# zhengyk19/vit-rpe-rope

Measured on AMD Instinct MI355X. Metric: train images/sec, CIFAR-10 ViT d=192 L=6 H=6, higher is better.
Workload: dtype bf16; 1 GPU; CIFAR-10-shaped 32x32 patch4 ViT d=192 L=6 H=6, --pos_encoding rope-axial theta=100, bf16, full train step (fwd+CE+bwd+AdamW), random-init weights; per_gpu_batch=512, global_batch=512, parallelism=dp1, hip_graph=True

## Files before the change

include/vitpe_debug.h:

```cpp
#ifndef VITPE_DEBUG_H
#define VITPE_DEBUG_H
#include "vitpe.h"
#ifdef __cplusplus
extern "C" {
#endif

int vitpe_selftest_mma(int dtype, const void* A, const void* Bt, const void* Brow, float* C_row,
                       float* C_tr, vitpe_stream_t stream);

int vitpe_debug_wgrad_census(int dtype, const vitpe_wgrad_problem* problems, int nprob, unsigned long long* census,
                             vitpe_stream_t stream);
int vitpe_debug_attn_census(const void* xn, const void* wqkv, void* out, const float* cos, const float* sin,
                            int B, unsigned long long* census, vitpe_stream_t stream);
int vitpe_debug_attn32_census(const void* xn, const void* wqkv_wide, void* out, const float* cos, const float* sin,
                              int B, unsigned long long* census, vitpe_stream_t stream);
int vitpe_debug_tail2_census(const void* attn_out, const void* x_in, const void* Wp_packed, const float* bp,
                             const float* gamma, const float* beta, void* x_mid, float* mean2, float* rstd2,
                             void* xn_out, const void* W1_packed, const float* b1, const void* W2_packed,
                             const float* b2, void* gp_out, void* h_out, void* out, float* mean_out, float* rstd_out,
                             int M, int HID, unsigned long long* census, vitpe_stream_t stream);
int vitpe_debug_set_gemm2d_mt(int mt);
int vitpe_debug_set_wgrad_wide(int on);
int vitpe_debug_read_bw(const void* src, long long bytes, int depth, int workgroups, unsigned* sink, vitpe_stream_t stream);
#ifdef __cplusplus
}
#endif
#endif
```

vit-rpe-rope_amd/csrc/wgrad.hip:

```cpp
#include "common.h"
#include <stdlib.h>

namespace vitpe {

constexpr int WG_MAXPROB = 28;
constexpr int WG_BLK = 192;

struct WgProb {
  const void* dY;
  const void* X;
  float* dW;
  float* dbias;
  const float* xmean;
  const float* xrstd;
  const float* xgamma;
  const float* xbeta;
  int M, N, K;
  int xop;
  int rs;
  int unit0;
  int nbn;
  int stages;
};
constexpr int WG_TABLE = 512;
struct WgArgs {
  int nprob, total_units, units_per_wg;
  int use_table;
  int nranges;
  int full_rounds, total_blocks;
  int tail_rounds;
  int bk;
  int nbig;
  int short_slots;
  int range_major;
  unsigned long long* census;
  WgProb p[WG_MAXPROB];
  unsigned short table[WG_TABLE];
};
static_assert(sizeof(WgArgs) <= 4096, "kernel argument block");
constexpr int WG_CENSUS_STAGES = 24, WG_CENSUS_SLOTS = 4;
constexpr int WG_SHORT_SPR = 2;

template <typename T> struct WgLayout;
template <> struct WgLayout<bf16> {
  static constexpr int LD = WG_BLK;
  static __device__ __forceinline__ int chunk(int r, int cc) {
    const int s = ((r >> 1) & 1) | (((r >> 3) & 1) << 1);
    return r * LD + ((((cc >> 1) ^ s)) << 4) + ((cc & 1) << 3);
  }
  static __device__ __forceinline__ Frag<bf16> tr(const bf16* tile, int rb0, int rb1, int c0) { return tr_ld<LD>(tile, rb0, rb1, c0); }
  template <int LD>
  static __device__ __forceinline__ Frag<bf16> tr_ld(const bf16* tile, int rb0, int rb1, int c0) {
    const int i = threadIdx.x & 15, q = i >> 2, p = i & 3;
    typedef __attribute__((address_space(3))) s16x4 lds_s16x4;
    const int r0 = rb0 + q, r1 = rb1 + q;
    constexpr int PAR = (LD % 128 == 0) ? 4 : 0;
    const int s0 = (((r0 >> 1) & 1) | (((r0 >> 3) & 1) << 1)) ^ ((r0 & 1) * PAR), s1 = (((r1 >> 1) & 1) | (((r1 >> 3) & 1) << 1)) ^ ((r1 & 1) * PAR);
    const bf16* a0 = tile + r0 * LD + (((c0 >> 4) ^ s0) << 4) + 4 * p;
    const bf16* a1 = tile + r1 * LD + (((c0 >> 4) ^ s1) << 4) + 4 * p;
    s16x4 lo = __builtin_amdgcn_ds_read_tr16_b64_v4i16((lds_s16x4*)a0);
    s16x4 hi = __builtin_amdgcn_ds_read_tr16_b64_v4i16((lds_s16x4*)a1);
    const s16x8 both = __builtin_shufflevector(lo, hi, 0, 1, 2, 3, 4, 5, 6, 7);
    Frag<bf16> f;
    f.v = __builtin_bit_cast(bf16x8, both);
    return f;
  }
};
template <> struct WgLayout<float> {
  static constexpr int LD = WG_BLK + 4;
  static __device__ __forceinline__ int chunk(int r, int cc) { return r * LD + cc * 4; }
  static __device__ __forceinline__ Frag<float> tr(const float* tile, int rb0, int rb1, int c0) {
    return ld_frag_tr(tile, LD, rb0, rb1, c0);
  }
};

template <class RunFn>
VITPE_DEV void wg_dispatch_placed(const WgArgs& a, RunFn run);

template <class RunFn>
VITPE_DEV void wg_dispatch(const WgArgs& a, RunFn run) {
  wg_dispatch_placed(a, run);
  for (int s = blockIdx.x; s < a.short_slots; s += gridDim.x) {
    int q = s, pi = a.nbig;
    for (int i = a.nbig; i < a.nprob - 1; ++i) {
      const int nsl = a.p[i].nbn * ((a.p[i].K + a.bk - 1) / a.bk) * ((a.p[i].stages + WG_SHORT_SPR - 1) / WG_SHORT_SPR);
      if (pi == i && q >= nsl) { q -= nsl; pi = i + 1; }
    }
    const WgProb& P = a.p[pi];
    const int nr = (P.stages + WG_SHORT_SPR - 1) / WG_SHORT_SPR;
    const int ub = P.unit0 + (q / nr) * P.stages, u0 = ub + (q % nr) * WG_SHORT_SPR;
    run(u0, min(ub + P.stages, u0 + WG_SHORT_SPR));
  }
}

template <class RunFn>
VITPE_DEV void wg_dispatch_placed(const WgArgs& a, RunFn run) {
  if (a.use_table == 2) {
    const int G = gridDim.x, idx = (blockIdx.x & 7) * (G >> 3) + (blockIdx.x >> 3);
    const int nrounds = a.range_major ? a.full_rounds : a.full_rounds + a.tail_rounds;
    for (int r = 0; r < nrounds; ++r) {
      int gb, rng = 0, R = 1;
      if (a.range_major) {
        const int vb = r * G + idx;
        R = a.nranges;
        rng = vb / a.total_blocks;
        gb = rng < R ? vb - rng * a.total_blocks : a.total_blocks;
      } else if (r < a.full_rounds) {
        gb = r * G + idx;
      } else {
        R = a.nranges;
        const int rem = a.total_blocks - a.full_rounds * G, q = (r - a.full_rounds) * G + idx;
        if (q >= rem * R) continue;
        rng = q / rem;
        gb = a.full_rounds * G + q % rem;
      }
      if (gb >= a.total_blocks) continue;
      int pi = 0, b0 = 0;
      for (int i = 0; i < a.nbig; ++i) {
        const int nb = a.p[i].nbn * ((a.p[i].K + a.bk - 1) / a.bk);
        if (gb >= b0 + nb) { b0 += nb; pi = i + 1; } else break;
      }
      const WgProb& P = a.p[pi];
      const int spr = (P.stages + R - 1) / R;
      const int ub = P.unit0 + (gb - b0) * P.stages;
      const int u0 = ub + min(P.stages, rng * spr), uend = ub + min(P.stages, (rng + 1) * spr);
      if (u0 < uend) run(u0, uend);
    }
    return;
  }
  int u0, uend;
  if (a.use_table == 1) {
    const unsigned ent = a.table[blockIdx.x];
    if (ent == 0xFFFFu) return;
    const WgProb& P = a.p[ent >> 11];
    const int blk = (int)((ent >> 5) & 0x3Fu), rng = (int)(ent & 0x1Fu);
    const int spr = (P.stages + a.nranges - 1) / a.nranges;
    u0 = P.unit0 + blk * P.stages + min(P.stages, rng * spr);
    uend = P.unit0 + blk * P.stages + min(P.stages, (rng + 1) * spr);
  } else {
    u0 = blockIdx.x * a.units_per_wg;
    uend = min(a.total_units, u0 + a.units_per_wg);
  }
  if (u0 >= uend) return;
  run(u0, uend);
}

template <typename T, bool CENSUS, bool LNX>
__global__ __launch_bounds__(768) void wgrad_group_kernel(WgArgs a) {
  using LY = WgLayout<T>;
  constexpr int RPS = 128 / (int)sizeof(T);
  constexpr int CPS = RPS / 32;
  constexpr int CHN = CH<T>::n;
  constexpr int CPR = WG_BLK / CHN;
  static_assert(RPS * CPR == 2 * 768, "a slab is two chunks per thread");
  constexpr int SLAB = RPS * LY::LD;
  __shared__ __attribute__((aligned(16))) T sm[2 * 2 * SLAB];

  const int tid = threadIdx.x, lane = tid & 63, c = lane & 15, g = lane >> 4;
  const int wave = __builtin_amdgcn_readfirstlane(tid >> 6);
  const int wn = wave / 3, wk = wave % 3;

  struct Cur {
    const T* dY; const T* X; float* dW; float* dbias;
    const float* xmean; const float* xrstd; const float* xgamma; const float* xbeta;
    int M, N, K, n0, k0, stage, stages, xop, rs;
  };
  auto decode = [&](int u, Cur& s) {
    int pi = 0;
    for (int i = 1; i < a.nprob; ++i) pi = (u >= a.p[i].unit0) ? i : pi;
    const WgProb& P = a.p[pi];
    const int ub = u - P.unit0, blk = ub / P.stages;
    s.dY = reinterpret_cast<const T*>(P.dY); s.X = reinterpret_cast<const T*>(P.X); s.dW = P.dW; s.dbias = P.dbias;
    s.M = P.M; s.N = P.N; s.K = P.K; s.stages = P.stages;
    s.xmean = P.xop ? P.xmean : reinterpret_cast<const float*>(P.dY);
    s.xrstd = P.xop ? P.xrstd : reinterpret_cast<const float*>(P.dY);
    s.xgamma = P.xgamma; s.xbeta = P.xbeta; s.xop = P.xop; s.rs = P.rs;
    s.stage = ub - blk * P.stages;
    s.n0 = (blk % P.nbn) * WG_BLK;
    s.k0 = (blk / P.nbn) * a.bk;
  };

  const Chunk16 zero = {0u, 0u, 0u, 0u};
  Chunk16 rg[4];
  float lnA[2], lnB[2];
  bool ln_staged = false;
  auto gload = [&](const Cur& s) {
    const int mb = s.stage * RPS;
    ln_staged = LNX && s.xop == 1;
#pragma unroll
    for (int i = 0; i < 4; ++i) {
      const int q = tid + 768 * (i & 1), row = q / CPR, cc = q % CPR;
      const int gm = mb + row;
      if (i < 2) {
        const int gn = s.n0 + cc * CHN;
        rg[i] = (gm < s.M && gn < s.N) ? *reinterpret_cast<const Chunk16*>(s.dY + (size_t)gm * s.rs * s.N + gn) : zero;
      } else {
        const int gk = s.k0 + cc * CHN;
        const bool ok = gm < s.M && gk < s.K;
        rg[i] = ok ? *reinterpret_cast<const Chunk16*>(s.X + (size_t)gm * s.rs * s.K + gk) : zero;
        if (LNX) {
          const size_t gs = (s.xop == 1) ? (size_t)min(gm, s.M - 1) * s.rs : 0;
          lnA[i - 2] = s.xrstd[gs];
          lnB[i - 2] = s.xmean[gs];
        }
      }
    }
  };
  auto sstore = [&](int buf) {
#pragma unroll
    for (int i = 0; i < 4; ++i) {
      const int q = tid + 768 * (i & 1), row = q / CPR, cc = q % CPR;
      Chunk16 v = rg[i];
      if (LNX && i >= 2 && ln_staged) {
        float f[CHN];
        chunk_to_f32<T>(v, f);
        const float rs = lnA[i - 2], nb = -lnB[i - 2] * rs;
#pragma unroll
        for (int t = 0; t < CHN; ++t) f[t] = fmaf(f[t], rs, nb);
        v = f32_to_chunk<T>(f);
      }
      *reinterpret_cast<Chunk16*>(sm + (buf * 2 + (i >> 1)) * SLAB + LY::chunk(row, cc)) = v;
    }
  };

  f32x4 acc[3][4], accb[3];
  auto clear = [&]() {
#pragma unroll
    for (int nt = 0; nt < 3; ++nt) {
      accb[nt] = (f32x4){0.f, 0.f, 0.f, 0.f};
#pragma unroll
      for (int kt = 0; kt < 4; ++kt) acc[nt][kt] = (f32x4){0.f, 0.f, 0.f, 0.f};
    }
  };
  Frag<T> ones;
#pragma unroll
  for (int t = 0; t < 8; ++t) ones.v[t] = from_f32<T>(1.0f);

  auto compute = [&](int buf, bool bias) {
    const T* sY = sm + (buf * 2 + 0) * SLAB;
    const T* sX = sm + (buf * 2 + 1) * SLAB;
#pragma unroll
    for (int cs = 0; cs < CPS; ++cs) {
      const int rb0 = cs * 32 + 8 * g, rb1 = rb0 + 4;
      Frag<T> fy[3], fx[4];
#pragma unroll
      for (int nt = 0; nt < 3; ++nt) fy[nt] = LY::tr(sY, rb0, rb1, wn * 48 + 16 * nt);
#pragma unroll
      for (int kt = 0; kt < 4; ++kt) fx[kt] = LY::tr(sX, rb0, rb1, wk * 64 + 16 * kt);
#pragma unroll
      for (int nt = 0; nt < 3; ++nt)
#pragma unroll
        for (int kt = 0; kt < 4; ++kt) mma(fy[nt], fx[kt], acc[nt][kt]);
      if (bias) {
#pragma unroll
        for (int nt = 0; nt < 3; ++nt) mma(fy[nt], ones, accb[nt]);
      }
    }
  };
  auto flush = [&](const Cur& s, bool bias) {
    float gam[4], bet[4];
#pragma unroll
    for (int kt = 0; kt < 4; ++kt) {
      const int gk = s.k0 + wk * 64 + 16 * kt + c;
      gam[kt] = (LNX && s.xop == 1 && gk < s.K) ? s.xgamma[gk] : 1.f;
      bet[kt] = (LNX && s.xop == 1 && gk < s.K) ? s.xbeta[gk] : 0.f;
    }
#pragma unroll
    for (int nt = 0; nt < 3; ++nt)
#pragma unroll
      for (int r = 0; r < 4; ++r) {
        const int gn = s.n0 + wn * 48 + 16 * nt + 4 * g + r;
#pragma unroll
        for (int kt = 0; kt < 4; ++kt) {
          const int gk = s.k0 + wk * 64 + 16 * kt + c;
          float v = acc[nt][kt][r];
          if (LNX && s.xop == 1) v = fmaf(v, gam[kt], bet[kt] * accb[nt][r]);
          if (gn < s.N && gk < s.K) atomicAdd(s.dW + (size_t)gn * s.K + gk, v);
        }
        if (bias && c == 0 && gn < s.N) atomicAdd(s.dbias + gn, accb[nt][r]);
      }
    clear();
  };

  bool first_run = true;
  auto run = [&](int u0, int uend) {
    if (!first_run) __syncthreads();
    first_run = false;
  Cur cur, nxt;
    decode(u0, cur);
    gload(cur);
    clear();
    auto stamp = [&](int u, int slot) {
      if (CENSUS && lane == 0 && u - u0 < WG_CENSUS_STAGES)
        a.census[(((size_t)blockIdx.x * 12 + wave) * WG_CENSUS_STAGES + (u - u0)) * WG_CENSUS_SLOTS + slot] = __builtin_amdgcn_s_memtime();
    };
    for (int u = u0; u < uend; ++u) {
      const int buf = (u - u0) & 1;
      sstore(buf);
      stamp(u, 0);
      nxt = cur;
      bool flush_now = (u + 1 == uend);
      if (u + 1 < uend) {
        if (cur.stage + 1 < cur.stages) nxt.stage = cur.stage + 1;
        else { decode(u + 1, nxt); flush_now = true; }
        gload(nxt);
      }
      stamp(u, 2);
      __syncthreads();
      stamp(u, 1);
      const bool bias = (cur.dbias != nullptr) && cur.k0 == 0 && wk == 0;
      compute(buf, bias || (LNX && cur.xop == 1));
      stamp(u, 3);
      if (flush_now) flush(cur, bias);
      cur = nxt;
    }
  };

  wg_dispatch(a, run);
}

constexpr int WW_BK = 384, WW_TH = 512;

__global__ __launch_bounds__(WW_TH) void wgrad_wide_kernel(WgArgs a) {
  using T = bf16;
  using LY = WgLayout<bf16>;
  constexpr int RPS = 64, YLD = WG_BLK, XLD = WW_BK;
  constexpr int YSLAB = RPS * YLD, XSLAB = RPS * XLD, STG = YSLAB + XSLAB;
  constexpr int YI = YSLAB / 512, XI = XSLAB / 512, NI = (YI + XI) / 8;
  static_assert((YI + XI) % 8 == 0, "instructions per wave");
  __shared__ __attribute__((aligned(1024))) T sm[2 * STG];

  const int tid = threadIdx.x, lane = tid & 63, c = lane & 15, g = lane >> 4;
  const int wave = __builtin_amdgcn_readfirstlane(tid >> 6);
  const int wn = wave >> 2, wk = wave & 3;

  struct Cur { const T* dY; const T* X; float* dW; float* dbias; int M, N, K, n0, k0, stage, stages; };
  auto decode = [&](int u, Cur& s) {
    int pi = 0;
    for (int i = 1; i < a.nprob; ++i) pi = (u >= a.p[i].unit0) ? i : pi;
    const WgProb& P = a.p[pi];
    const int ub = u - P.unit0, blk = ub / P.stages;
    s.dY = reinterpret_cast<const T*>(P.dY); s.X = reinterpret_cast<const T*>(P.X); s.dW = P.dW; s.dbias = P.dbias;
    s.M = P.M; s.N = P.N; s.K = P.K; s.stages = P.stages;
    s.stage = ub - blk * P.stages;
    s.n0 = (blk % P.nbn) * WG_BLK;
    s.k0 = (blk / P.nbn) * WW_BK;
  };
  auto swz = [](int r, int cl) { return ((((cl >> 1) ^ (((r >> 1) & 1) | (((r >> 3) & 1) << 1))) << 1) | (cl & 1)); };
  auto swzx = [](int r, int cl) {
    return ((((cl >> 1) ^ ((((r >> 1) & 1) | (((r >> 3) & 1) << 1)) ^ ((r & 1) << 2))) << 1) | (cl & 1));
  };
  static_assert(YI == 24 && XI == 48, "instruction j of a wave: j < 3 -> dY slab, else X slab");
  const unsigned sm_lds = (unsigned)(uintptr_t)(__attribute__((address_space(3))) void*)sm;
  auto dma = [&](const Cur& s, int buf) {
    const int mb = s.stage * RPS;
    int ln = lane;
    asm volatile("" : "+v"(ln));
#pragma unroll
    for (int j = 0; j < NI; ++j) {
      const int q = wave + 8 * j;
      const T* src;
      if (j < 3) {
        const int p = q * 64 + ln, r = p / (YLD / 8), cl = p % (YLD / 8);
        src = s.dY + (size_t)min(mb + r, s.M - 1) * s.N + s.n0 + swz(r, cl) * 8;
      } else {
        const int p = (q - YI) * 64 + ln, r = p / (XLD / 8), cl = p % (XLD / 8);
        src = s.X + (size_t)min(mb + r, s.M - 1) * s.K + s.k0 + swzx(r, cl) * 8;
      }
      const unsigned dst = sm_lds + (unsigned)(buf * STG + q * 512) * 2;
      unsigned keep;
      asm volatile("s_mov_b32 %0, m0\n\ts_mov_b32 m0, %2\n\ts_nop 0\n\tglobal_load_lds_dwordx4 %1, off\n\ts_mov_b32 m0, %0"
                   : "=&s"(keep) : "v"(src), "s"(dst) : "memory");
    }
  };

  f32x4 acc[6][6], accb[2];
  auto clear = [&]() {
    accb[0] = accb[1] = (f32x4){0.f, 0.f, 0.f, 0.f};
#pragma unroll
    for (int nt = 0; nt < 6; ++nt)
#pragma unroll
      for (int kt = 0; kt < 6; ++kt) acc[nt][kt] = (f32x4){0.f, 0.f, 0.f, 0.f};
  };
  Frag<T> ones;
#pragma unroll
  for (int t = 0; t < 8; ++t) ones.v[t] = from_f32<T>(1.0f);

  auto compute = [&](int buf, bool bias) {
    const T* sY = sm + buf * STG;
    const T* sX = sY + YSLAB;
#pragma unroll
    for (int cs = 0; cs < 2; ++cs) {
      const int rb0 = cs * 32 + 8 * g, rb1 = rb0 + 4;
      __builtin_amdgcn_sched_barrier(0);
      Frag<T> fy[6];
#pragma unroll
      for (int nt = 0; nt < 6; ++nt) fy[nt] = LY::tr_ld<YLD>(sY, rb0, rb1, wn * 96 + 16 * nt);
#pragma unroll
      for (int h = 0; h < 2; ++h) {
        Frag<T> fx[3];
#pragma unroll
        for (int t = 0; t < 3; ++t) fx[t] = LY::tr_ld<XLD>(sX, rb0, rb1, wk * 96 + 16 * (3 * h + t));
#pragma unroll
        for (int nt = 0; nt < 6; ++nt)
#pragma unroll
          for (int t = 0; t < 3; ++t) mma(fy[nt], fx[t], acc[nt][3 * h + t]);
        __builtin_amdgcn_sched_barrier(0);
      }
      if (bias) {
        if (wk == 0) { mma(fy[0], ones, accb[0]); mma(fy[1], ones, accb[1]); }
        else if (wk == 1) { mma(fy[2], ones, accb[0]); mma(fy[3], ones, accb[1]); }
        else { mma(fy[4], ones, accb[0]); mma(fy[5], ones, accb[1]); }
      }
    }
  };
  auto flush = [&](const Cur& s, bool bias) {
#pragma unroll
    for (int nt = 0; nt < 6; ++nt)
#pragma unroll
      for (int r = 0; r < 4; ++r) {
        const int gn = s.n0 + wn * 96 + 16 * nt + 4 * g + r;
        float* row = s.dW + (size_t)gn * s.K + s.k0 + wk * 96 + c;
#pragma unroll
        for (int kt = 0; kt < 6; ++kt) atomicAdd(row + 16 * kt, acc[nt][kt][r]);
      }
    if (bias && c == 0) {
#pragma unroll
      for (int t = 0; t < 2; ++t)
#pragma unroll
        for (int r = 0; r < 4; ++r) atomicAdd(s.dbias + s.n0 + wn * 96 + 16 * (2 * wk + t) + 4 * g + r, accb[t][r]);
    }
    clear();
  };

  bool first_run = true;
  auto run = [&](int u0, int uend) {
    if (!first_run) __syncthreads();
    first_run = false;
    Cur cur, nxt;
    decode(u0, cur);
    dma(cur, 0);
    clear();
    for (int u = u0; u < uend; ++u) {
      const int buf = (u - u0) & 1;
      __builtin_amdgcn_s_waitcnt(0x0F70);
      __syncthreads();
      if (cur.stage * RPS + RPS > cur.M) {
        const int first = cur.M - cur.stage * RPS;
        T* sY = sm + buf * STG;
        for (int q = tid; q < (RPS - first) * (YLD / 8); q += WW_TH)
          *reinterpret_cast<Chunk16*>(sY + first * YLD + q * 8) = (Chunk16){0u, 0u, 0u, 0u};
        __syncthreads();
      }
      nxt = cur;
      bool flush_now = (u + 1 == uend);
      if (u + 1 < uend) {
        if (cur.stage + 1 < cur.stages) nxt.stage = cur.stage + 1;
        else { decode(u + 1, nxt); flush_now = true; }
        dma(nxt, buf ^ 1);
      }
      const bool bias = (cur.dbias != nullptr) && cur.k0 == 0 && wk < 3;
      compute(buf, bias);
      if (flush_now) flush(cur, bias);
      cur = nxt;
    }
  };
  wg_dispatch(a, run);
}

}

using namespace vitpe;

struct vitpe_wgrad_problem_abi {
  const void* dY;
  const void* X;
  float* dW;
  float* dbias;
  int M, N, K, x_op;
  const float* x_mean;
  const float* x_rstd;
  const float* x_gamma;
  const float* x_beta;
};

static int wgrad_cu_count() {
  static int n = 0;
  if (n == 0) {
    int dev = 0, v = 0;
    if (hipGetDevice(&dev) != hipSuccess || hipDeviceGetAttribute(&v, hipDeviceAttributeMultiprocessorCount, dev) != hipSuccess || v <= 0)
      v = 256;
    n = v;
  }
  return n;
}

static int wgrad_group_launch(int dtype, const void* problems, const int* row_step, int nprob, unsigned long long* census,
                              hipStream_t stream);
static bool g_wide_ok = true;
extern "C" int vitpe_debug_set_wgrad_wide(int on) { g_wide_ok = on != 0; return 0; }

extern "C" int vitpe_wgrad_group(int dtype, const void* problems, int nprob, hipStream_t stream) {
  return wgrad_group_launch(dtype, problems, nullptr, nprob, nullptr, stream);
}

extern "C" int vitpe_wgrad_group_rows(int dtype, const void* problems, const int* row_step, int nprob, hipStream_t stream) {
  return wgrad_group_launch(dtype, problems, row_step, nprob, nullptr, stream);
}

extern "C" int vitpe_debug_wgrad_census(int dtype, const void* problems, int nprob, unsigned long long* census,
                                        hipStream_t stream) {
  VITPE_REQUIRE(census != nullptr && dtype == 1);
  return wgrad_group_launch(dtype, problems, nullptr, nprob, census, stream);
}

static int wgrad_group_launch(int dtype, const void* problems, const int* row_step, int nprob, unsigned long long* census,
                              hipStream_t stream) {
  VITPE_REQUIRE(problems && nprob >= 0 && nprob <= WG_MAXPROB && (dtype == 0 || dtype == 1));
  const vitpe_wgrad_problem_abi* pr = reinterpret_cast<const vitpe_wgrad_problem_abi*>(problems);
  const int RPS = dtype == 1 ? 64 : 32, CHN = dtype == 1 ? 8 : 4;
  WgArgs a{};
  a.census = census;
  bool wide = g_wide_ok && dtype == 1 && census == nullptr && nprob > 0;
  for (int i = 0; i < nprob; ++i)
    wide = wide && (pr[i].M == 0 || (pr[i].x_op == 0 && pr[i].N % WG_BLK == 0 && pr[i].K % WW_BK == 0 &&
                                     (row_step == nullptr || row_step[i] <= 1)));
  a.bk = wide ? WW_BK : WG_BLK;
  int max_stages = 0;
  for (int i = 0; i < nprob; ++i) max_stages = (pr[i].M + RPS - 1) / RPS > max_stages ? (pr[i].M + RPS - 1) / RPS : max_stages;
  int units = 0, np = 0, nbig = 0;
  for (int pass = 0; pass < 2; ++pass) {
    for (int i = 0; i < nprob; ++i) {
      const vitpe_wgrad_problem_abi& p = pr[i];
      VITPE_REQUIRE(p.dY && p.X && p.dW && p.M >= 0 && p.N > 0 && p.K > 0 && p.N % CHN == 0 && p.K % CHN == 0);
      VITPE_REQUIRE(row_step == nullptr || row_step[i] >= 1);
      if (p.M == 0) continue;
      const int stages = (p.M + RPS - 1) / RPS;
      if ((stages * 8 <= max_stages) != (pass == 1)) continue;
      WgProb& q = a.p[np++];
      VITPE_REQUIRE(p.x_op == 0 || (p.x_op == 1 && p.x_mean && p.x_rstd && p.x_gamma && p.x_beta));
      q.dY = p.dY; q.X = p.X; q.dW = p.dW; q.dbias = p.dbias; q.M = p.M; q.N = p.N; q.K = p.K;
      q.xop = p.x_op; q.xmean = p.x_mean; q.xrstd = p.x_rstd; q.xgamma = p.x_gamma; q.xbeta = p.x_beta;
      q.rs = row_step != nullptr ? row_step[i] : 1;
      q.unit0 = units;
      q.nbn = (p.N + WG_BLK - 1) / WG_BLK;
      q.stages = stages;
      const long long nu = (long long)q.nbn * ((p.K + a.bk - 1) / a.bk) * q.stages;
      VITPE_REQUIRE(units + nu < (1LL << 30));
      units += (int)nu;
    }
    if (pass == 0) nbig = np;
  }
  if (units == 0) return 0;
  a.nprob = np;
  a.nbig = nbig;
  a.total_units = units;
  const int np_all = np;
  np = nbig;
  const int ncu = wgrad_cu_count();
  int grid = 0;
  int total_blocks = 0, max_blocks = 0, min_stages = 1 << 30;
  for (int i = 0; i < np; ++i) {
    const int nb = a.p[i].nbn * ((a.p[i].K + a.bk - 1) / a.bk);
    total_blocks += nb;
    max_blocks = nb > max_blocks ? nb : max_blocks;
    min_stages = a.p[i].stages < min_stages ? a.p[i].stages : min_stages;
  }
  int R = (2 * ncu) / (total_blocks > 0 ? total_blocks : 1);
  if (R > 255) R = 255;
  if (R >= 2 && R <= 8 && R <= min_stages / 4 && max_blocks <= 63 && np <= 31) {
    int len[8] = {0, 0, 0, 0, 0, 0, 0, 0};
    bool fits = true;
    for (int i = 0; i < WG_TABLE; ++i) a.table[i] = 0xFFFFu;
    for (int r = 0; r < R && fits; ++r)
      for (int i = 0; i < np && fits; ++i) {
        const int nb = a.p[i].nbn * ((a.p[i].K + a.bk - 1) / a.bk);
        int x = 0;
        for (int k = 1; k < 8; ++k) x = len[k] < len[x] ? k : x;
        for (int b = 0; b < nb; ++b) {
          const int id = (len[x] + b) * 8 + x;
          if (id >= WG_TABLE) { fits = false; break; }
          a.table[id] = (unsigned short)(((unsigned)i << 11) | ((unsigned)b << 5) | (unsigned)r);
        }
        len[x] += nb;
      }
    if (fits) {
      int mx = 0;
      for (int k = 0; k < 8; ++k) mx = len[k] > mx ? len[k] : mx;
      a.use_table = 1;
      a.nranges = R;
      grid = mx * 8;
    }
  }
  const int G = ncu & ~7;
  if (!a.use_table && G >= 8 && total_blocks >= G) {
    a.use_table = 2;
    a.total_blocks = total_blocks;
    a.full_rounds = total_blocks / G;
    const int rem = total_blocks - a.full_rounds * G;
    int bestR = 1, bestT = rem > 0 ? 1 : 0;
    int Rmax = min_stages / 4;
    if (Rmax > 8) Rmax = 8;
    for (int Rc = 2; rem > 0 && Rc <= Rmax; ++Rc) {
      const int Tc = (rem * Rc + G - 1) / G;
      if ((long long)Tc * bestR < (long long)bestT * Rc) { bestR = Rc; bestT = Tc; }
    }
    a.nranges = bestR;
    a.tail_rounds = bestT;
    grid = G;
  }
  if (!a.use_table && G >= 8 && total_blocks > 0 && total_blocks < G) {
    int bestR = 0, bestk = 0;
    double besteff = 0.0;
    for (int k = 1; k <= 3; ++k) {
      int Rk = (k * G) / total_blocks;
      if (Rk > min_stages / 4) Rk = min_stages / 4;
      if (Rk > 31) Rk = 31;
      if (Rk < 2) continue;
      const double eff = (double)total_blocks * Rk / (double)(((total_blocks * Rk + G - 1) / G) * G);
      if (eff > besteff + 1e-9) { besteff = eff; bestR = Rk; bestk = k; }
    }
    if (bestR >= 2 && besteff >= 0.97) {
      a.use_table = 2;
      a.range_major = 1;
      a.total_blocks = total_blocks;
      a.nranges = bestR;
      a.full_rounds = (total_blocks * bestR + G - 1) / G;
      grid = G;
      (void)bestk;
    }
  }
  if (a.use_table) {
    for (int i = nbig; i < np_all; ++i)
      a.short_slots += a.p[i].nbn * ((a.p[i].K + a.bk - 1) / a.bk) * ((a.p[i].stages + WG_SHORT_SPR - 1) / WG_SHORT_SPR);
  }
  np = np_all;
  if (!a.use_table) {
    const int wgs = units < ncu ? units : ncu;
    a.units_per_wg = (units + wgs - 1) / wgs;
    grid = (units + a.units_per_wg - 1) / a.units_per_wg;
  }
  bool lnx = false;
  for (int i = 0; i < np; ++i) lnx = lnx || a.p[i].xop != 0;
  if (census != nullptr) VITPE_REQUIRE(!lnx && dtype == 1);
  if (wide) hipLaunchKernelGGL(wgrad_wide_kernel, dim3(grid), dim3(WW_TH), 0, stream, a);
  else if (census != nullptr) hipLaunchKernelGGL((wgrad_group_kernel<bf16, true, false>), dim3(grid), dim3(768), 0, stream, a);
  else if (dtype == 1 && lnx) hipLaunchKernelGGL((wgrad_group_kernel<bf16, false, true>), dim3(grid), dim3(768), 0, stream, a);
  else if (dtype == 1) hipLaunchKernelGGL((wgrad_group_kernel<bf16, false, false>), dim3(grid), dim3(768), 0, stream, a);
  else if (lnx) hipLaunchKernelGGL((wgrad_group_kernel<float, false, true>), dim3(grid), dim3(768), 0, stream, a);
  else hipLaunchKernelGGL((wgrad_group_kernel<float, false, false>), dim3(grid), dim3(768), 0, stream, a);
  VITPE_CHECK_LAUNCH();
}
```

vit-rpe-rope_amd/vitpe/engine.py:

```python
from __future__ import annotations

import contextlib
import dataclasses
import math
import os
from typing import Dict, List, Optional

import numpy as np
import torch
import torch.distributed as dist
import torch.nn as nn

from . import _lib as L
from . import ddp
from . import kernels as K
from .positional_encoding import (AbsolutePositionalEncoding, PolynomialRPE, RelativePositionalEncoding, RoPEAxial,
                                  RoPEMixed)
from .head import StepHead
from .optim import StepOptimizer
from .route import (ALIGN, KIND_FRAG, KIND_FRAG_PHI, KIND_QKV, KIND_QKV_WIDE, KIND_T, Route, resolve_route,
                    shadow_plan)
from .vit import VisionTransformer

SITE_ATTN, SITE_PROJ, SITE_MLP1, SITE_MLP2, SITE_PATH_A, SITE_PATH_M = range(6)
SITES_PER_LAYER = 6


def site_row(layer: int, site: int) -> int:
    return SITES_PER_LAYER * layer + site


def shift_rng_offsets(table: torch.Tensor, rank: int) -> torch.Tensor:
    inc = (int(rank) << 48) & 0xFFFFFFFFFFFFFFFF
    out = table.clone()
    out[:, 1] += inc - (1 << 64) if inc >= (1 << 63) else inc
    return out


def new_augment_rng(device, rank: int = 0) -> torch.Tensor:
    return shift_rng_offsets(K.new_rng_pairs(1, device), rank)


def engine_unsupported(model):
    active = []
    for blk in model.blocks:
        if blk.attn.qkv.bias is not None:
            active.append("qkv_bias")
        if blk.attn.attn_drop_p > 0.:
            active.append("attn_drop")
        if blk.attn.proj_drop_p > 0. or blk.mlp.drop > 0.:
            active.append("drop")
        if blk.drop_path_p > 0.:
            active.append("drop_path")
    return sorted(set(active))


class TrainEngine:
    def __init__(self, model: VisionTransformer, batch_size: int, compute_dtype=torch.bfloat16, lr=1e-3,
                 weight_decay=0.01, betas=(0.9, 0.999), eps=1e-8, process_group=None, use_graph=True, fuse_ln=None,
                 extras=False):
        active = engine_unsupported(model)
        if active and not extras:
            raise NotImplementedError("TrainEngine does not support " + ", ".join(active) + " (the fused training path has "
                                      "no qkv bias and no dropout); train this model through the module path instead.  "
                                      "TrainEngine(..., extras=True) runs them on the per-Linear route")
        dev = next(model.parameters()).device
        if dev.type != "cuda":
            raise L.VitpeError("TrainEngine needs the model on the HIP device (no CPU path)")
        self.model, self.dev, self.T, self.B = model, dev, compute_dtype, batch_size
        self.pg = process_group
        self.world = dist.get_world_size(process_group) if (dist.is_available() and dist.is_initialized()) else 1
        self.use_graph = use_graph
        m = model
        self.D, self.H, self.Lyr, self.p = m.embed_dim, m.num_heads, len(m.blocks), m.patch_size
        self.C, self.P, self.Cn = m.patch_embed.weight.shape[1], m.num_patches, m.num_classes
        self.N, self.grid = self.P + 1, int(math.sqrt(self.P))
        self.S, self.M = self.grid * self.p, self.B * self.N
        self.hid = m.blocks[0].mlp.fc1.weight.shape[0]
        self.route: Route = resolve_route(compute_dtype, self.C, self.S, self.p, self.D, self.H, self.hid, self.Lyr, self.Cn,
                                          extras=extras, fuse_ln=fuse_ln)
        self.__dict__.update(dataclasses.asdict(self.route))
        self._save_hidden = True
        self._build_flat(lr, weight_decay, betas, eps)
        self._build_buffers()
        self._build_rng_table()
        self.aug_rng, self.aug_pad, self.aug_hflip = None, 0, False
        self.split_layer = max(1, self.Lyr // 2)
        self.bucket_off = self._off[id(next(self.model.blocks[self.split_layer].parameters()))] \
            if self.Lyr >= 2 else 0
        self.overlap_comm = self.world > 1 and self.Lyr >= 2
        self.allpairs = (ddp.AllPairsSum(self.pg) if self.world > 1 and os.environ.get("VITPE_DDP_ALLPAIRS", "0") == "1"
                         else None)
        self._comm_stream = torch.cuda.Stream(device=dev) if self.allpairs is not None else None
        self.ddp_graph = self.world > 1 and os.environ.get("VITPE_DDP_GRAPH", "0") == "1"
        self._drop_graphs()
        self.steps_done = 0

    def _drop_graphs(self):
        self.graph_fb = self.graph_fb2 = self.graph_opt = None

    def _rank(self) -> int:
        return dist.get_rank(self.pg) if self.world > 1 else 0

    def _build_flat(self, lr, wd, betas, eps):
        params = list(self.model.parameters())
        starts, n = ddp.flat_layout([prm.numel() for prm in params], ALIGN)
        offs = {id(prm): o for prm, o in zip(params, starts)}
        self.n_flat = n
# ... 473 lines not shown

    def _part_layers(self, part):
        top, split = self.Lyr - 1, self.split_layer
        return {"all": (top, 0), "upper": (top, split), "lower": (split - 1, 0)}[part]

    def _wgrad_group(self, part):
        if part not in self._wg_groups:
            hi, lo = self._part_layers(part)
            probs = [p for l in range(hi, lo - 1, -1) for p in self._wgrad_problems(l).values()]
            if part != "upper":
                probs.append(self._embed_wgrad())
            ng = -(-len(probs) // K.WgradGroup.MAX)
            per = -(-len(probs) // ng)
            self._wg_groups[part] = [K.WgradGroup(probs[i:i + per]) for i in range(0, len(probs), per)]
        for grp in self._wg_groups[part]:
            grp.launch()

    def _gemm_tn(self, l, name):
        if not self.group_wgrad:
            K.gemm_tn(*self._wgrad_problems(l)[name])

    def _backward(self, part="all"):
        mdl, G = self.model, self.Gr
        hi, lo = self._part_layers(part)
        if part != "lower" and not self.fuse_head:
            self.head.backward()
        for l in range(hi, lo - 1, -1):
            self._layer_bwd(l, lo, hi)
        if part != "upper":
            dape = None
            if isinstance(mdl.pos_embed, AbsolutePositionalEncoding):
                dape = G(mdl.pos_embed.pos_embed)[0, :self.P]
            K.embed_bwd(self.dx_out[0], G(mdl.cls_token).view(-1), dape, out=self.dpatch)
            if not self.group_wgrad:
                K.gemm_tn(*self._embed_wgrad())
        if self.group_wgrad:
            self._wgrad_group(part)

    def _optimizer(self):
        self.opt.launch(self.head.ticked)
        self.head.ticked = False
        self.refresh_shadows(cast_flat=False)
        if self.extras:
            K.rng_advance(self.rng_table, 1)
        if self.aug_rng is not None:
            K.rng_advance(self.aug_rng, 1)

    def _allreduce(self):
        if self.allpairs is not None:
            self.allpairs(self.flat_g)
        else:
            ddp.allreduce_sum_(self.flat_g, self.pg)

    def set_valid(self, n_valid: int, n_valid_global: Optional[int] = None):
        self.head.set_valid(n_valid, n_valid_global)

    def sync_from_model(self):
        self.refresh_shadows()

    def broadcast_parameters(self, src=0):
        if self.world > 1:
            ddp.broadcast_(self.flat_p, src, self.pg)
            self.refresh_shadows()
        if self.opt.ema_decay is not None:
            self.reset_ema()

    def capture(self):
        self.opt.guard("capture")
        state = [self.flat_p, *self.head.state_tensors(), *self.opt.state_tensors(),
                 *(t for t in (self.rng_table, self.aug_rng) if t is not None)]
        snap = [t.clone() for t in state]
        s = torch.cuda.Stream()
        s.wait_stream(torch.cuda.current_stream())
        with torch.cuda.stream(s):
            for _ in range(2):
                self._fwd_train(); self._loss(); self._backward(); self._optimizer()
        torch.cuda.current_stream().wait_stream(s)
        torch.cuda.synchronize()
        for t, c in zip(state, snap):
            t.copy_(c)
        self.flat_g.zero_()
        self.refresh_shadows()
        torch.cuda.synchronize()
        if self.ddp_graph:
            try:
                g = torch.cuda.CUDAGraph()
                with torch.cuda.graph(g, capture_error_mode="thread_local"):
                    self._fwd_train(); self._loss()
                    if self.overlap_comm:
                        self._backward("upper")
                        side, main = torch.cuda.Stream(), torch.cuda.current_stream()
                        side.wait_stream(main)
                        with torch.cuda.stream(side):
                            dist.all_reduce(self.flat_g[self.bucket_off:], op=dist.ReduceOp.SUM, group=self.pg)
                        self._backward("lower")
                        dist.all_reduce(self.flat_g[:self.bucket_off], op=dist.ReduceOp.SUM, group=self.pg)
                        main.wait_stream(side)
                    else:
                        self._backward()
                        self._allreduce()
                    self._optimizer()
                torch.cuda.synchronize()
                self.graph_fb, self.graph_fb2, self.graph_opt = g, None, None
                return
            except Exception as exc:
                import warnings
                warnings.warn(f"VITPE_DDP_GRAPH: capturing the all-reduces failed ({exc!r}); using the host-stitched step")
                self.ddp_graph = False
                torch.cuda.synchronize()
                self.flat_g.zero_()
        self.graph_fb = torch.cuda.CUDAGraph()
        with torch.cuda.graph(self.graph_fb, capture_error_mode="thread_local"):
            self._fwd_train(); self._loss()
            if self.world == 1:
                self._backward(); self._optimizer()
            elif self.overlap_comm:
                self._backward("upper")
            else:
                self._backward()
        if self.world > 1:
            if self.overlap_comm:
                self.graph_fb2 = torch.cuda.CUDAGraph()
                with torch.cuda.graph(self.graph_fb2, capture_error_mode="thread_local"):
                    self._backward("lower")
            self.graph_opt = torch.cuda.CUDAGraph()
            with torch.cuda.graph(self.graph_opt, capture_error_mode="thread_local"):
                self._optimizer()
        torch.cuda.synchronize()

    def attach_dataset(self, dataset):
        if dataset is self.dataset:
            return
        if dataset is not None:
            C, S = dataset.images.shape[1], dataset.images.shape[2]
            if (C, S) != (self.C, self.S) or dataset.images.device != self.dev:
                raise L.VitpeError(f"dataset is {C}x{S}x{S} on {dataset.images.device}, engine expects "
                                   f"{self.C}x{self.S}x{self.S} on {self.dev}")
            if self.batch_idx is None:
                self.batch_idx = torch.zeros(self.B, dtype=torch.int64, device=self.dev)
        self.dataset = dataset
        self._drop_graphs()

    def _load_indices(self, idx: torch.Tensor, dataset=None):
        dataset = dataset if dataset is not None else self.dataset
        if dataset is None:
            raise L.VitpeError("no dataset attached (TrainEngine.attach_dataset)")
        n = idx.shape[0] if idx.dim() == 1 else -1
        if not (1 <= n <= self.B) or idx.dtype != torch.int64:
            raise L.VitpeError(f"expected 1..{self.B} int64 sample indices, got {tuple(idx.shape)} {idx.dtype}")
        if n < self.B:
            self.batch_idx.fill_(idx[0])
            self.batch_idx[:n].copy_(idx, non_blocking=True)
        else:
            self.batch_idx.copy_(idx, non_blocking=True)
        torch.index_select(dataset.labels, 0, self.batch_idx, out=self.labels)
        return n

    def step_indexed(self, idx: torch.Tensor, n_valid_global: Optional[int] = None, n_valid: Optional[int] = None):
        self.opt.guard("step_indexed")
        n = self._load_indices(idx)
        self.set_valid(n if n_valid is None else min(n, n_valid), n_valid_global)
        self.step()

    def forward_indexed(self, idx: torch.Tensor, dataset=None) -> torch.Tensor:
        keep = self.dataset
        if dataset is not None:
# ... 167 lines not shown
```

Baseline: 380,100 images/sec.

## Fuse short wgrad slots into placed runs and transpose atomic flush via permlane

Replaces the callback-based wgrad dispatch with an iterator that lets each workgroup chain its placed big-problem run and trailing short-problem slots without re-priming the pipeline. In range-major mode it shortens the last ranges by a slot cost so short slots can be absorbed behind them. It also raises short-slot size from 2 to 8 stages. The flush now transposes 4x4 accumulator fragments with permlane swaps so the atomicAdds hit contiguous columns, at the cost of added s_nop padding. Graph capture also runs with Python GC paused, and a host-side debug routine enumerates runs.

Result: no change. 382,000 images/sec, median of 3 (+0.5%).

```diff
diff --git a/include/vitpe_debug.h b/include/vitpe_debug.h
--- a/include/vitpe_debug.h
+++ b/include/vitpe_debug.h
@@ -10,6 +10,8 @@
 
 int vitpe_debug_wgrad_census(int dtype, const vitpe_wgrad_problem* problems, int nprob, unsigned long long* census,
                              vitpe_stream_t stream);
+int vitpe_debug_wgrad_runs(int dtype, const vitpe_wgrad_problem* problems, const int* row_step, int nprob, int ncu,
+                           int* info, int* prob_info, int* runs, int max_runs);
 int vitpe_debug_attn_census(const void* xn, const void* wqkv, void* out, const float* cos, const float* sin,
                             int B, unsigned long long* census, vitpe_stream_t stream);
 int vitpe_debug_attn32_census(const void* xn, const void* wqkv_wide, void* out, const float* cos, const float* sin,
diff --git a/vit-rpe-rope_amd/csrc/wgrad.hip b/vit-rpe-rope_amd/csrc/wgrad.hip
--- a/vit-rpe-rope_amd/csrc/wgrad.hip
+++ b/vit-rpe-rope_amd/csrc/wgrad.hip
@@ -33,13 +33,16 @@
   int nbig;
   int short_slots;
   int range_major;
+  int short_spr;
+  int slot_cost;
   unsigned long long* census;
   WgProb p[WG_MAXPROB];
   unsigned short table[WG_TABLE];
 };
 static_assert(sizeof(WgArgs) <= 4096, "kernel argument block");
 constexpr int WG_CENSUS_STAGES = 24, WG_CENSUS_SLOTS = 4;
-constexpr int WG_SHORT_SPR = 2;
+constexpr int WG_SHORT_SPR = 8;
+constexpr int WG_SLOT_FLUSH = 5;
 
 template <typename T> struct WgLayout;
 template <> struct WgLayout<bf16> {
@@ -74,31 +77,40 @@
   }
 };
 
-template <class RunFn>
-VITPE_DEV void wg_dispatch_placed(const WgArgs& a, RunFn run);
-
-template <class RunFn>
-VITPE_DEV void wg_dispatch(const WgArgs& a, RunFn run) {
-  wg_dispatch_placed(a, run);
-  for (int s = blockIdx.x; s < a.short_slots; s += gridDim.x) {
-    int q = s, pi = a.nbig;
-    for (int i = a.nbig; i < a.nprob - 1; ++i) {
-      const int nsl = a.p[i].nbn * ((a.p[i].K + a.bk - 1) / a.bk) * ((a.p[i].stages + WG_SHORT_SPR - 1) / WG_SHORT_SPR);
-      if (pi == i && q >= nsl) { q -= nsl; pi = i + 1; }
-    }
-    const WgProb& P = a.p[pi];
-    const int nr = (P.stages + WG_SHORT_SPR - 1) / WG_SHORT_SPR;
-    const int ub = P.unit0 + (q / nr) * P.stages, u0 = ub + (q % nr) * WG_SHORT_SPR;
-    run(u0, min(ub + P.stages, u0 + WG_SHORT_SPR));
-  }
-}
-
-template <class RunFn>
-VITPE_DEV void wg_dispatch_placed(const WgArgs& a, RunFn run) {
+struct WgRunIter {
+  int round = 0;
+  int pend = -1;
+  int slot = 0;
+};
+#define VITPE_HD __host__ __device__ __forceinline__
+VITPE_HD int wg_min(int x, int y) { return x < y ? x : y; }
+VITPE_HD int wg_max(int x, int y) { return x > y ? x : y; }
+
+VITPE_HD void wg_slot_run(const WgArgs& a, int s, int& u0, int& uend) {
+  int q = s, pi = a.nbig;
+  for (int i = a.nbig; i < a.nprob - 1; ++i) {
+    const int nsl = a.p[i].nbn * ((a.p[i].K + a.bk - 1) / a.bk) * ((a.p[i].stages + a.short_spr - 1) / a.short_spr);
+    if (pi == i && q >= nsl) { q -= nsl; pi = i + 1; }
+  }
+  const WgProb& P = a.p[pi];
+  const int nr = (P.stages + a.short_spr - 1) / a.short_spr;
+  const int ub = P.unit0 + (q / nr) * P.stages;
+  u0 = ub + (q % nr) * a.short_spr;
+  uend = wg_min(ub + P.stages, u0 + a.short_spr);
+}
+
+VITPE_HD bool wg_next_run(const WgArgs& a, int wg, int G, WgRunIter& it, int& u0, int& uend) {
+  if (it.pend >= 0) {
+    wg_slot_run(a, it.pend, u0, uend);
+    it.pend = -1;
+    return true;
+  }
+  const bool behind = a.range_major && a.slot_cost > 0;
   if (a.use_table == 2) {
-    const int G = gridDim.x, idx = (blockIdx.x & 7) * (G >> 3) + (blockIdx.x >> 3);
+    const int idx = (wg & 7) * (G >> 3) + (wg >> 3);
     const int nrounds = a.range_major ? a.full_rounds : a.full_rounds + a.tail_rounds;
-    for (int r = 0; r < nrounds; ++r) {
+    while (it.round < nrounds) {
+      const int r = it.round++;
       int gb, rng = 0, R = 1;
       if (a.range_major) {
         const int vb = r * G + idx;
@@ -121,28 +133,54 @@
         if (gb >= b0 + nb) { b0 += nb; pi = i + 1; } else break;
       }
       const WgProb& P = a.p[pi];
-      const int spr = (P.stages + R - 1) / R;
       const int ub = P.unit0 + (gb - b0) * P.stages;
-      const int u0 = ub + min(P.stages, rng * spr), uend = ub + min(P.stages, (rng + 1) * spr);
-      if (u0 < uend) run(u0, uend);
-    }
-    return;
-  }
-  int u0, uend;
-  if (a.use_table == 1) {
-    const unsigned ent = a.table[blockIdx.x];
-    if (ent == 0xFFFFu) return;
-    const WgProb& P = a.p[ent >> 11];
-    const int blk = (int)((ent >> 5) & 0x3Fu), rng = (int)(ent & 0x1Fu);
-    const int spr = (P.stages + a.nranges - 1) / a.nranges;
-    u0 = P.unit0 + blk * P.stages + min(P.stages, rng * spr);
-    uend = P.unit0 + blk * P.stages + min(P.stages, (rng + 1) * spr);
-  } else {
-    u0 = blockIdx.x * a.units_per_wg;
-    uend = min(a.total_units, u0 + a.units_per_wg);
-  }
-  if (u0 >= uend) return;
-  run(u0, uend);
+      const int ns = behind ? wg_max(0, wg_min(R, (a.short_slots - gb + a.total_blocks - 1) / a.total_blocks)) : 0;
+      const int spr = (P.stages + ns * a.slot_cost + R - 1) / R;
+      const int s0 = rng * spr - a.slot_cost * wg_max(0, rng - (R - ns));
+      const int s1 = rng + 1 == R ? P.stages : (rng + 1) * spr - a.slot_cost * wg_max(0, rng + 1 - (R - ns));
+      u0 = ub + wg_min(P.stages, s0);
+      uend = ub + wg_min(P.stages, s1);
+      const int s = behind ? (R - 1 - rng) * a.total_blocks + gb : a.short_slots;
+      if (u0 < uend) {
+        it.pend = s < a.short_slots ? s : -1;
+        return true;
+      }
+      if (s < a.short_slots) {
+        wg_slot_run(a, s, u0, uend);
+        return true;
+      }
+    }
+  } else if (it.round == 0) {
+    it.round = 1;
+    u0 = uend = 0;
+    if (a.use_table == 1) {
+      const unsigned ent = a.table[wg];
+      if (ent != 0xFFFFu) {
+        const WgProb& P = a.p[ent >> 11];
+        const int blk = (int)((ent >> 5) & 0x3Fu), rng = (int)(ent & 0x1Fu);
+        const int spr = (P.stages + a.nranges - 1) / a.nranges;
+        u0 = P.unit0 + blk * P.stages + wg_min(P.stages, rng * spr);
+        uend = P.unit0 + blk * P.stages + wg_min(P.stages, (rng + 1) * spr);
+      }
+    } else {
+      u0 = wg * a.units_per_wg;
+      uend = wg_min(a.total_units, u0 + a.units_per_wg);
+    }
+    if (u0 < uend) return true;
+  }
+  const int first = behind ? wg_min(a.short_slots, a.nranges * a.total_blocks) : 0;
+  const int s = first + wg + it.slot * G;
+  if (s >= a.short_slots) return false;
+  ++it.slot;
+  wg_slot_run(a, s, u0, uend);
+  return true;
+}
+
+VITPE_DEV void wg_xpose4(float (&w)[4]) {
+  asm volatile("s_nop 1\n\tv_permlane16_swap_b32 %0, %1" : "+v"(w[0]), "+v"(w[1]));
+  asm volatile("s_nop 1\n\tv_permlane16_swap_b32 %0, %1" : "+v"(w[2]), "+v"(w[3]));
+  asm volatile("s_nop 1\n\tv_permlane32_swap_b32 %0, %1" : "+v"(w[0]), "+v"(w[2]));
+  asm volatile("s_nop 1\n\tv_permlane32_swap_b32 %0, %1" : "+v"(w[1]), "+v"(w[3]));
 }
 
 template <typename T, bool CENSUS, bool LNX>
@@ -265,31 +303,43 @@
       gam[kt] = (LNX && s.xop == 1 && gk < s.K) ? s.xgamma[gk] : 1.f;
       bet[kt] = (LNX && s.xop == 1 && gk < s.K) ? s.xbeta[gk] : 0.f;
     }
+    __builtin_amdgcn_sched_barrier(0);
+    asm volatile("s_nop 15\n\ts_nop 15");
+    __builtin_amdgcn_sched_barrier(0);
 #pragma unroll
     for (int nt = 0; nt < 3; ++nt)
 #pragma unroll
       for (int r = 0; r < 4; ++r) {
         const int gn = s.n0 + wn * 48 + 16 * nt + 4 * g + r;
+        float w[4];
 #pragma unroll
         for (int kt = 0; kt < 4; ++kt) {
-          const int gk = s.k0 + wk * 64 + 16 * kt + c;
-          float v = acc[nt][kt][r];
-          if (LNX && s.xop == 1) v = fmaf(v, gam[kt], bet[kt] * accb[nt][r]);
-          if (gn < s.N && gk < s.K) atomicAdd(s.dW + (size_t)gn * s.K + gk, v);
+          w[kt] = acc[nt][kt][r];
+          if (LNX && s.xop == 1) w[kt] = fmaf(w[kt], gam[kt], bet[kt] * accb[nt][r]);
+        }
+        wg_xpose4(w);
+        const int gk = s.k0 + wk * 64 + 16 * g + c;
+#pragma unroll
+        for (int j = 0; j < 4; ++j) {
+          const int gr = s.n0 + wn * 48 + 16 * nt + 4 * j + r;
+          if (gr < s.N && gk < s.K) atomicAdd(s.dW + (size_t)gr * s.K + gk, w[j]);
         }
         if (bias && c == 0 && gn < s.N) atomicAdd(s.dbias + gn, accb[nt][r]);
+        __builtin_amdgcn_sched_barrier(0);
       }
     clear();
   };
 
-  bool first_run = true;
-  auto run = [&](int u0, int uend) {
-    if (!first_run) __syncthreads();
-    first_run = false;
+  WgRunIter it;
+  int u0, uend;
+  if (!wg_next_run(a, (int)blockIdx.x, (int)gridDim.x, it, u0, uend)) return;
   Cur cur, nxt;
-    decode(u0, cur);
-    gload(cur);
-    clear();
+  decode(u0, cur);
+  gload(cur);
+  clear();
+  for (;;) {
+    int n0 = 0, nend = 0;
+    const bool more = wg_next_run(a, (int)blockIdx.x, (int)gridDim.x, it, n0, nend);
     auto stamp = [&](int u, int slot) {
       if (CENSUS && lane == 0 && u - u0 < WG_CENSUS_STAGES)
         a.census[(((size_t)blockIdx.x * 12 + wave) * WG_CENSUS_STAGES + (u - u0)) * WG_CENSUS_SLOTS + slot] = __builtin_amdgcn_s_memtime();
@@ -299,12 +349,12 @@
       sstore(buf);
       stamp(u, 0);
       nxt = cur;
-      bool flush_now = (u + 1 == uend);
-      if (u + 1 < uend) {
-        if (cur.stage + 1 < cur.stages) nxt.stage = cur.stage + 1;
-        else { decode(u + 1, nxt); flush_now = true; }
-        gload(nxt);
-      }
+      const bool last = (u + 1 == uend);
+      const bool go_on = !last || more;
+      bool flush_now = last;
+      if (!last && cur.stage + 1 < cur.stages) nxt.stage = cur.stage + 1;
+      else if (go_on) { decode(last ? n0 : u + 1, nxt); flush_now = true; }
+      if (go_on) gload(nxt);
       stamp(u, 2);
       __syncthreads();
       stamp(u, 1);
@@ -314,9 +364,11 @@
       if (flush_now) flush(cur, bias);
       cur = nxt;
     }
-  };
-
-  wg_dispatch(a, run);
+    if (!more) break;
+    __syncthreads();
+    u0 = n0;
+    uend = nend;
+  }
 }
 
 constexpr int WW_BK = 384, WW_TH = 512;
@@ -433,10 +485,10 @@
     clear();
   };
 
-  bool first_run = true;
-  auto run = [&](int u0, int uend) {
+  WgRunIter it;
+  int u0, uend;
+  for (bool first_run = true; wg_next_run(a, (int)blockIdx.x, (int)gridDim.x, it, u0, uend); first_run = false) {
     if (!first_run) __syncthreads();
-    first_run = false;
     Cur cur, nxt;
     decode(u0, cur);
     dma(cur, 0);
@@ -464,8 +516,7 @@
       if (flush_now) flush(cur, bias);
       cur = nxt;
     }
-  };
-  wg_dispatch(a, run);
+  }
 }
 
 }
@@ -514,13 +565,15 @@
   return wgrad_group_launch(dtype, problems, nullptr, nprob, census, stream);
 }
 
-static int wgrad_group_launch(int dtype, const void* problems, const int* row_step, int nprob, unsigned long long* census,
-                              hipStream_t stream) {
+static int wgrad_place(int dtype, const void* problems, const int* row_step, int nprob, unsigned long long* census, int ncu,
+                       WgArgs& a, int& grid, bool& wide_out, int* source) {
+  grid = 0;
   VITPE_REQUIRE(problems && nprob >= 0 && nprob <= WG_MAXPROB && (dtype == 0 || dtype == 1));
   const vitpe_wgrad_problem_abi* pr = reinterpret_cast<const vitpe_wgrad_problem_abi*>(problems);
   const int RPS = dtype == 1 ? 64 : 32, CHN = dtype == 1 ? 8 : 4;
-  WgArgs a{};
+  a = WgArgs{};
   a.census = census;
+  a.short_spr = WG_SHORT_SPR;
   bool wide = g_wide_ok && dtype == 1 && census == nullptr && nprob > 0;
   for (int i = 0; i < nprob; ++i)
     wide = wide && (pr[i].M == 0 || (pr[i].x_op == 0 && pr[i].N % WG_BLK == 0 && pr[i].K % WW_BK == 0 &&
@@ -537,6 +590,7 @@
       if (p.M == 0) continue;
       const int stages = (p.M + RPS - 1) / RPS;
       if ((stages * 8 <= max_stages) != (pass == 1)) continue;
+      if (source != nullptr) source[np] = i;
       WgProb& q = a.p[np++];
       VITPE_REQUIRE(p.x_op == 0 || (p.x_op == 1 && p.x_mean && p.x_rstd && p.x_gamma && p.x_beta));
       q.dY = p.dY; q.X = p.X; q.dW = p.dW; q.dbias = p.dbias; q.M = p.M; q.N = p.N; q.K = p.K;
@@ -557,8 +611,6 @@
   a.total_units = units;
   const int np_all = np;
   np = nbig;
-  const int ncu = wgrad_cu_count();
-  int grid = 0;
   int total_blocks = 0, max_blocks = 0, min_stages = 1 << 30;
   for (int i = 0; i < np; ++i) {
     const int nb = a.p[i].nbn * ((a.p[i].K + a.bk - 1) / a.bk);
@@ -632,7 +684,13 @@
   }
   if (a.use_table) {
     for (int i = nbig; i < np_all; ++i)
-      a.short_slots += a.p[i].nbn * ((a.p[i].K + a.bk - 1) / a.bk) * ((a.p[i].stages + WG_SHORT_SPR - 1) / WG_SHORT_SPR);
+      a.short_slots += a.p[i].nbn * ((a.p[i].K + a.bk - 1) / a.bk) * ((a.p[i].stages + a.short_spr - 1) / a.short_spr);
+    if (a.range_major && a.short_slots > 0) {
+      int cost = 0;
+      for (int i = nbig; i < np_all; ++i) cost = a.p[i].stages > cost ? a.p[i].stages : cost;
+      cost = (cost < a.short_spr ? cost : a.short_spr) + WG_SLOT_FLUSH;
+      a.slot_cost = cost < min_stages / a.nranges ? cost : min_stages / a.nranges;
+    }
   }
   np = np_all;
   if (!a.use_table) {
@@ -640,8 +698,46 @@
     a.units_per_wg = (units + wgs - 1) / wgs;
     grid = (units + a.units_per_wg - 1) / a.units_per_wg;
   }
+  wide_out = wide;
+  return 0;
+}
+
+extern "C" int vitpe_debug_wgrad_runs(int dtype, const void* problems, const int* row_step, int nprob, int ncu, int* info,
+                                      int* prob_info, int* runs, int max_runs) {
+  VITPE_REQUIRE(info && prob_info && runs && ncu > 0 && max_runs >= 0);
+  WgArgs a;
+  int grid = 0, source[WG_MAXPROB];
+  bool wide = false;
+  const int err = wgrad_place(dtype, problems, row_step, nprob, nullptr, ncu, a, grid, wide, source);
+  if (err != 0) return err;
+  int n = 0;
+  for (int wg = 0; wg < grid; ++wg) {
+    WgRunIter it;
+    int u0, uend;
+    while (wg_next_run(a, wg, grid, it, u0, uend)) {
+      VITPE_REQUIRE(n < max_runs);
+      runs[3 * n] = wg; runs[3 * n + 1] = u0; runs[3 * n + 2] = uend;
+      ++n;
+    }
+  }
+  const int vals[10] = {grid, n, a.use_table, a.range_major, wide ? 1 : 0, a.nranges, a.total_units, a.short_slots, a.nprob, a.slot_cost};
+  for (int i = 0; i < 10; ++i) info[i] = vals[i];
+  for (int i = 0; i < a.nprob; ++i) {
+    prob_info[4 * i] = source[i]; prob_info[4 * i + 1] = a.p[i].unit0;
+    prob_info[4 * i + 2] = a.p[i].nbn * ((a.p[i].K + a.bk - 1) / a.bk); prob_info[4 * i + 3] = a.p[i].stages;
+  }
+  return 0;
+}
+
+static int wgrad_group_launch(int dtype, const void* problems, const int* row_step, int nprob, unsigned long long* census,
+                              hipStream_t stream) {
+  WgArgs a;
+  int grid = 0;
+  bool wide = false;
+  const int err = wgrad_place(dtype, problems, row_step, nprob, census, wgrad_cu_count(), a, grid, wide, nullptr);
+  if (err != 0 || grid == 0) return err;
   bool lnx = false;
-  for (int i = 0; i < np; ++i) lnx = lnx || a.p[i].xop != 0;
+  for (int i = 0; i < a.nprob; ++i) lnx = lnx || a.p[i].xop != 0;
   if (census != nullptr) VITPE_REQUIRE(!lnx && dtype == 1);
   if (wide) hipLaunchKernelGGL(wgrad_wide_kernel, dim3(grid), dim3(WW_TH), 0, stream, a);
   else if (census != nullptr) hipLaunchKernelGGL((wgrad_group_kernel<bf16, true, false>), dim3(grid), dim3(768), 0, stream, a);
diff --git a/vit-rpe-rope_amd/vitpe/engine.py b/vit-rpe-rope_amd/vitpe/engine.py
--- a/vit-rpe-rope_amd/vitpe/engine.py
+++ b/vit-rpe-rope_amd/vitpe/engine.py
@@ -2,6 +2,7 @@
 
 import contextlib
 import dataclasses
+import gc
 import math
 import os
 from typing import Dict, List, Optional
@@ -24,6 +25,18 @@
 
 SITE_ATTN, SITE_PROJ, SITE_MLP1, SITE_MLP2, SITE_PATH_A, SITE_PATH_M = range(6)
 SITES_PER_LAYER = 6
+
+
+@contextlib.contextmanager
+def _gc_paused():
+    gc.collect()
+    was_enabled = gc.isenabled()
+    gc.disable()
+    try:
+        yield
+    finally:
+        if was_enabled:
+            gc.enable()
 
 
 def site_row(layer: int, site: int) -> int:
@@ -663,6 +676,10 @@
         self.flat_g.zero_()
         self.refresh_shadows()
         torch.cuda.synchronize()
+        with _gc_paused():
+            self._capture_graphs()
+
+    def _capture_graphs(self):
         if self.ddp_graph:
             try:
                 g = torch.cuda.CUDAGraph()
```
